# SerezD/vqvae-vqgan-pytorch-lightning

Measured on AMD Instinct MI355X. Metric: images/sec/node (256x256 bs=32/GPU) VQ-VAE train step, higher is better.
Workload: dtype bf16; 1 GPU; standard_vqvae cb=1024, 256x256 bs=32/GPU (encoder+VQ+decoder fwd/bwd + AdamW); yaml=example_confs/standard_vqvae.yaml, global_batch=32, parallelism=dp1, launch=hipGraph replay (fwd+bwd) + eager all-reduce + AdamW, deterministic=False

## Files before the change

### vqvae-vqgan-pytorch-lightning_amd/csrc/api.cpp

```cpp
#include <stdint.h>
#include <new>
#include "common.h"

extern "C" {

const char* vqk_status_str(int status) {
    switch (status) {
        case VQK_OK: return "ok";
        case VQK_ERR_SHAPE: return "unsupported or inconsistent shape";
        case VQK_ERR_DTYPE: return "unsupported dtype";
        case VQK_ERR_ALIGN: return "pointer is not 16-byte aligned";
        case VQK_ERR_LAUNCH: return "kernel launch failed";
        case VQK_ERR_ARG: return "bad argument";
        case VQK_ERR_WORKSPACE: return "workspace too small";
        default: return "unknown status";
    }
}

int vqk_version(void) { return 1; }
const char* vqk_arch(void) { return "gfx950"; }

}

struct vqk_ctx {
    vqkd::DetState det, scratch, tq;
};
namespace vqkd {
static vqk_ctx& default_ctx() {
    static thread_local vqk_ctx c = {{0, nullptr, 0}, {0, nullptr, 0}, {0, nullptr, 0}};
    return c;
}
static vqk_ctx*& current_ctx() {
    static thread_local vqk_ctx* cur = nullptr;
    return cur;
}
static vqk_ctx& ctx() {
    vqk_ctx* c = current_ctx();
    return c ? *c : default_ctx();
}
DetState& det_state() { return ctx().det; }
DetState& scratch_state() { return ctx().scratch; }
DetState& tile_queue_state() { return ctx().tq; }
}

extern "C" int vqk_ctx_create(vqk_ctx** out) {
    if (!out) return VQK_ERR_ARG;
    *out = new (std::nothrow) vqk_ctx{{0, nullptr, 0}, {0, nullptr, 0}, {0, nullptr, 0}};
    return *out ? VQK_OK : VQK_ERR_WORKSPACE;
}

extern "C" int vqk_ctx_destroy(vqk_ctx* c) {
    if (c && vqkd::current_ctx() == c) vqkd::current_ctx() = nullptr;
    delete c;
    return VQK_OK;
}

extern "C" int vqk_ctx_make_current(vqk_ctx* c) {
    vqkd::current_ctx() = c;
    return VQK_OK;
}

extern "C" int vqk_ctx_set_tile_queue(vqk_ctx* c, void* ws, int64_t ws_bytes) {
    if (ws && ws_bytes < 64) return VQK_ERR_WORKSPACE;
    if (ws && (reinterpret_cast<uintptr_t>(ws) & 15)) return VQK_ERR_ALIGN;
    vqkd::DetState& d = c ? c->tq : vqkd::ctx().tq;
    d.on = ws ? 1 : 0;
    d.ws = reinterpret_cast<float*>(ws);
    d.bytes = ws ? ws_bytes : 0;
    return VQK_OK;
}

extern "C" int vqk_ctx_set_scratch(vqk_ctx* c, void* ws, int64_t ws_bytes) {
    if (ws && ws_bytes < 0) return VQK_ERR_ARG;
    if (ws && (reinterpret_cast<uintptr_t>(ws) & 15)) return VQK_ERR_ALIGN;
    vqkd::DetState& d = c ? c->scratch : vqkd::ctx().scratch;
    d.on = ws ? 1 : 0;
    d.ws = reinterpret_cast<float*>(ws);
    d.bytes = ws ? ws_bytes : 0;
    return VQK_OK;
}

extern "C" int vqk_ctx_set_deterministic(vqk_ctx* c, int on, void* ws, int64_t ws_bytes) {
    if (on && ws && ws_bytes < 0) return VQK_ERR_ARG;
    if (on && ws && (reinterpret_cast<uintptr_t>(ws) & 15)) return VQK_ERR_ALIGN;
    vqkd::DetState& d = c ? c->det : vqkd::ctx().det;
    d.on = on ? 1 : 0;
    d.ws = (on && ws) ? reinterpret_cast<float*>(ws) : nullptr;
    d.bytes = (on && ws) ? ws_bytes : 0;
    return VQK_OK;
}

extern "C" int vqk_set_tile_queue(void* ws, int64_t ws_bytes) { return vqk_ctx_set_tile_queue(nullptr, ws, ws_bytes); }
extern "C" int vqk_set_scratch(void* ws, int64_t ws_bytes) { return vqk_ctx_set_scratch(nullptr, ws, ws_bytes); }
extern "C" int vqk_set_deterministic(int on, void* ws, int64_t ws_bytes) { return vqk_ctx_set_deterministic(nullptr, on, ws, ws_bytes); }

#include <string.h>
#include <stdlib.h>
namespace vqkd {
static TuneSlot g_tune[] = {
    {"MX", 0, 0},
    {"MX_1X1", 0, 0},
    {"TW16", 0, 0},
    {"STREAM_BLOCKS", 0, 0},
    {"MX_MIN_TILES", 0, 0},
    {"FPROP_SPLITK", 0, 0},
    {"SK_BLOCKS", 0, 0},
    {"SK_MINSTEPS", 0, 0},
    {"SK_MAXMB", 0, 0},
    {"UPS_PHASE", 0, 0},
    {"WGRAD_BLOCKS", 0, 0},
    {"WGMX", 0, 0},
    {"WGRAD_GEN_BLOCKS", 0, 0},
    {"WGRAD_NO_PW16", 0, 0},
    {"WGRAD_NO_P16K", 0, 0},
    {"MX_HALF", 0, 0},
    {"MX_HALF_HW", 0, 0},
    {"UPFIRDN_TILE", 0, 0},
    {"GN_BLOCKS_REDUCE", 0, 0},
    {"GN_BLOCKS_APPLY", 0, 0},
    {"GN_NT_MB", 0, 0},
    {"GN_NO_SMALL", 0, 0},
    {"WGMX_COEF_E4", 0, 0},
    {"GN_CLUSTER_MAX_HW", 0, 0},
    {"COMM_CUS", 0, 0},
    {"MX_QUARTER", 0, 0},
    {"MX_S2", 0, 0},
    {"MX_S2_DGRAD_MIN", 0, 0},
    {"VQ_LDS", 0, 0},
    {"UPS_MERGE", 0, 0},
    {"TILE_QUEUE", 0, 0},
    {"X3_WL", 0, 0},
    {"X3_WGRAD_COEF_E4", 0, 0},
    {"X3_WGRAD_FOLD", 0, 0},
    {"X3_WGRAD_PHASE", 0, 0},
    {"X3_WGRAD_PHASE_CAP_PCT", 0, 0},
    {"X3_WGRAD_PHASE_COEF_E4", 0, 0},
    {"WGRAD_GROUP_LOAD_PCT", 0, 0},
    {"WGRAD_GROUP_MIN_PPS", 0, 0},
    {"MX_PHASE_U64", 0, 0}
};
static constexpr int kTune = (int)(sizeof(g_tune) / sizeof(g_tune[0]));
TuneSlot* tune_slot(const char* name) {
    for (int i = 0; i < kTune; ++i)
        if (strcmp(g_tune[i].name, name) == 0) return &g_tune[i];
    abort();
}
}

extern "C" int vqk_set_tuning(const char* name, int value) {
    if (!name) return VQK_ERR_ARG;
    for (int i = 0; i < vqkd::kTune; ++i)
        if (strcmp(vqkd::g_tune[i].name, name) == 0) {
            __atomic_store_n(&vqkd::g_tune[i].value, value, __ATOMIC_RELAXED);
            __atomic_store_n(&vqkd::g_tune[i].is_set, 1, __ATOMIC_RELEASE);
            return VQK_OK;
        }
    return VQK_ERR_ARG;
}

extern "C" int vqk_reset_tuning(void) {
    for (int i = 0; i < vqkd::kTune; ++i) __atomic_store_n(&vqkd::g_tune[i].is_set, 0, __ATOMIC_RELAXED);
    return VQK_OK;
}

extern "C" int vqk_tuning_count(void) { return vqkd::kTune; }

extern "C" const char* vqk_tuning_name(int i) { return (i >= 0 && i < vqkd::kTune) ? vqkd::g_tune[i].name : nullptr; }
```

### vqvae-vqgan-pytorch-lightning_amd/csrc/conv_geom.h

```cpp
#pragma once
#include "common.h"

namespace vqkd {

struct ConvGeom {
    int n, h_in, w_in, h, w, cin, cout, ks, ups;
    int stride, pad, zs, vh, vw;
    float acc_scale, out_gain;
    int pool;
    float pool_scale;
    int m;
    int sub, sub_py, sub_px, sub_h, sub_w, nkh, nkw, khl[2], kwl[2];
    int wrow_chunks;
    int cpt;
    int kchunks;
    int tiles_m, tiles_n;
    int unit64;
    double* gn_ws;
    int gn_cpg;
    int gn_part_nblk, gn_part_base;
    int ntap, tap_oy, tap_ox, src_s, src_a, src_b, dst_s, dst_a, dst_b;
    int tapw, dst_h, dst_w, s2;
    int phase_mode;
    int phase_rev;
    int dy_pool;
    int act;
    int* tq;
    int tq_mode;
    int fold;
};

__device__ __forceinline__ int xcd_remap(int bid, int total) {
    const int q = total >> 3, r = total & 7, xcd = bid & 7, k = bid >> 3;
    return (xcd < r ? xcd * (q + 1) : r * (q + 1) + (xcd - r) * q) + k;
}

__device__ __forceinline__ unsigned pack_bf16x2(float a, float b) {
    typedef __attribute__((ext_vector_type(2))) float f32x2;
    typedef __attribute__((ext_vector_type(2))) __bf16 bf16x2_t;
    const f32x2 v = {a, b};
    return __builtin_bit_cast(unsigned, __builtin_convertvector(v, bf16x2_t));
}

constexpr int MX_LDS_MAX = 160 * 1024;
constexpr int mx_phase_u64_lds(int twlog) {
    return 2 * ((((256 >> twlog) + 1) * ((1 << twlog) + 1) * 9 + 63) / 64) * 1024 + 256 * 272 + 1024 + 64;
}

int launch_conv3x3_mx(const void* x, const void* w, const float* bias, const void* res, void* y, const void* zeros,
                      const ConvGeom& g, int twlog, hipStream_t st);

int conv_make_geom(ConvGeom& g, int dtype, int n, int h_in, int w_in, int cin, int cout, int ksize, int ups);
}
enum ConvVariant : int {
    CONV_VARIANT_AUTO = -1,
    CONV_VARIANT_IM2COL = 0,
    CONV_VARIANT_HALO = 1,
    CONV_VARIANT_PLAIN_WEIGHTS = 2,
    CONV_VARIANT_BREG = 3,
    CONV_VARIANT_NO_HALF = 4,
    CONV_VARIANT_NO_MX = 5,
    CONV_VARIANT_MX = 6,
};
enum WgradDyPool : int {
    WGRAD_DY_PLAIN = 0,
    WGRAD_DY_POOLED = 1,
    WGRAD_DY_PHASE0 = 2,
    WGRAD_DY_PHASES = 6,
    WGRAD_DY_PHASES_SWAPPED = 7,
};
enum WgradOp : int {
    WGRAD_OP_PLAIN = 0,
    WGRAD_OP_POOLED_DY = 1,
    WGRAD_OP_UPS_PHASE = 2,
    WGRAD_OP_POOLED_DY_PHASE = 3,
    WGRAD_OP_FOLD = 4,
    WGRAD_OP_X3 = 5,
};
namespace vqkd {
int& conv_force_variant();
int& conv_wgrad_blocks();

bool conv3x3_x3_serves(const ConvGeom& g);
int launch_conv3x3_x3(const void* x, const void* w, const float* bias, const void* res, void* y, const void* zeros,
                      const ConvGeom& g, int act, int blocks_cap, hipStream_t st);
int launch_conv3x3_wgrad_x3(const void* x, const void* dy, float* dw, const ConvGeom& g, int tiles, int splits, int pps, hipStream_t st);

int launch_conv3x3_thin_out_f32(const float* x, const float* w, const float* bias, const float* res, float* y, int n, int h, int wd,
                                int cin, int act, float acc_scale, float out_gain, hipStream_t st);
int launch_conv3x3_thin_in_f32(const float* x, const float* w, const float* bias, float* y, int n, int h, int wd, int cout, hipStream_t st);
int thin_wgrad_rows(int h, int w);
int launch_conv3x3_wgrad_thin_f32(int mode, const float* wide, const float* thin, float* dw, int n, int h, int w, int cw, float scale,
                                  hipStream_t st);

int launch_conv3x3_wgrad_mx(const void* x, const void* dy, float* dw, const void* zeros, const ConvGeom& g, int tiles,
                            int splits, int pps, hipStream_t st, float* part = nullptr);

#define VQK_WGRAD_GROUP_MAX 16
struct WgradGroupLayer {
    const void* x; const void* dy; float* dw;
    int n, h, w, cin, cout;
    float scale;
    int blk0, tiles, pps;
    int own;
};
struct WgradGroupTable {
    int n_layers, pad_;
    WgradGroupLayer layer[VQK_WGRAD_GROUP_MAX];
};
int launch_conv3x3_wgrad_mx_group(const WgradGroupTable& tb, int blocks, const void* zeros, hipStream_t st);

}
```

### vqvae-vqgan-pytorch-lightning_amd/csrc/conv_wgrad.hip

```cpp
#include "conv_geom.h"
#include <math.h>

namespace {

using vqkd::ConvGeom;
using vqkd::xcd_remap;

__device__ __forceinline__ void glds16(const void* src, char* lds_wave_base) {
    __builtin_amdgcn_global_load_lds((const VQK_GLB void*)src, (VQK_LDS void*)lds_wave_base, 16, 0, 0);
}

template <typename T> struct WgradFrag;

template <> struct WgradFrag<bf16_raw> {
    static constexpr int KP = 64;
    static constexpr int ROWB = 256;
    __device__ static __forceinline__ bf16x8_t frag(const char* tile, int k0, int cbase, int lane) {
        const int i = lane & 15, grp = (lane >> 4) & 1, kgrp = lane >> 5;
        const int col = cbase + 16 * grp + 4 * (i & 3);
        const int row = k0 + 8 * kgrp + (i >> 2);
        const int lc = col >> 3;
        const char* p0 = tile + row * ROWB + ((lc ^ ((row & 3) << 2)) << 4) + ((col & 7) << 1);
        const char* p1 = p0 + 4 * ROWB;
        const s16x4 lo = __builtin_amdgcn_ds_read_tr16_b64_v4i16((VQK_LDS s16x4*)p0);
// ... 437 lines not shown
    const int tco = bx / tiles_ci, tci = bx - tco * tiles_ci;
    const int co0 = tco * 64, ci0 = tci * 64;
    const int pw = g.w >> 4, ph = g.h >> 3;
    const int total_patches = g.n * ph * pw;
    const int p_begin = by * patches_per_split;
    const int p_end = min(total_patches, p_begin + patches_per_split);
    if (p_begin >= p_end) return;

    const int wi = wave >> 1, wj = wave & 1;
    f32x16 acc[9];
#pragma unroll
    for (int t = 0; t < 9; ++t)
#pragma unroll
        for (int r = 0; r < 16; ++r) acc[t][r] = 0.0f;

    const int lrow = lane >> 2, lch = (lane & 3) * 8;
    unsigned dyoff[NDY], xoff[NX];
#pragma unroll
    for (int sl = 0; sl < NDY; ++sl) {
        const int q = wave + 4 * sl, half = q >> 3, prow = q & 7;
        dyoff[sl] = (unsigned)((((prow * g.w + lrow) * g.cout) + co0 + half * 32 + lch) * 2);
    }
#pragma unroll
    for (int sl = 0; sl < NX; ++sl) {
        const int r = wave + 4 * sl, half = r / 12, row = min((r % 12) * 16 + lrow, HROWS - 1);
        const int hy = row / HWD, hx = row - hy * HWD;
        xoff[sl] = (unsigned)((((hy * g.w_in + hx) * g.cin) + ci0 + half * 32 + lch) * 2);
    }
    struct PatchPos { int img, py0, px0; bool interior; const char* bdy; const char* bx; };
    auto decode = [&](int patch) -> PatchPos {
        PatchPos pp;
        pp.img = patch / (ph * pw);
        const int rem = patch - pp.img * (ph * pw);
        const int pyi = rem / pw, pxi = rem - pyi * pw;
        pp.py0 = pyi * 8; pp.px0 = pxi * PWD;
        pp.interior = !g.ups && pp.py0 >= 1 && pp.py0 + 8 < g.h && pp.px0 >= 1 && pp.px0 + PWD < g.w;
        const int64_t pix = ((int64_t)pp.img * g.h + pp.py0) * g.w + pp.px0;
        pp.bdy = reinterpret_cast<const char*>(dy + pix * g.cout);
        pp.bx = reinterpret_cast<const char*>(x + (pix - g.w - 1) * g.cin);
        return pp;
    };
    auto piece = [&](bool interior, int sl, const PatchPos& pp, char* st) {
        if (sl < NDY) {
            const int q = wave + 4 * sl;
            char* dst = st + (q >> 3) * DY_HALF + (q & 7) * 1024;
            if (interior || true) {
                glds16(pp.bdy + dyoff[sl], dst);
            }
        } else {
            const int r = wave + 4 * (sl - NDY), half = r / 12, pr = r % 12;
            char* dst = st + 2 * DY_HALF + half * X_HALF + pr * 1024;
            if (interior) {
                glds16(pp.bx + xoff[sl - NDY], dst);
            } else {
                const int row = min(pr * 16 + lrow, HROWS - 1);
                const int hy = row / HWD, hx = row - hy * HWD;
                const int iy = pp.py0 + hy - 1, ix = pp.px0 + hx - 1;
                const void* src = zeros;
                if (iy >= 0 && iy < g.h && ix >= 0 && ix < g.w)
                    src = x + (((int64_t)pp.img * g.h_in + (iy >> g.ups)) * g.w_in + (ix >> g.ups)) * g.cin + ci0 + half * 32 + lch;
                glds16(src, dst);
            }
        }
    };

    const int li = lane & 15, grp = (lane >> 4) & 1, kgrp = lane >> 5;
    const unsigned frag_lane = (unsigned)((li >> 2) * 64 + 32 * grp + 8 * (li & 3));
    const unsigned a_lane = (unsigned)(wi * DY_HALF) + frag_lane + (unsigned)(kgrp * 8 * 64);
    const unsigned b_lane = (unsigned)(2 * DY_HALF + wj * X_HALF) + frag_lane + (unsigned)(kgrp * 8 * 64);

    {
        const PatchPos p0 = decode(p_begin);
#pragma unroll
        for (int sl = 0; sl < NDY + NX; ++sl) piece(p0.interior, sl, p0, smem);
    }
    for (int pch = p_begin; pch < p_end; ++pch) {
        const unsigned cur = (unsigned)(((pch - p_begin) & 1) * STAGE);
        asm volatile("s_waitcnt vmcnt(0)" ::: "memory");
        __syncthreads();
        const bool has_next = pch + 1 < p_end;
        const PatchPos pp = decode(has_next ? pch + 1 : pch);
        char* nst = smem + (STAGE - cur);
        const char* pa = smem + cur + a_lane;
        const char* pb = smem + cur + b_lane;
        if (has_next) {
            if (pp.interior) {
#pragma unroll
                for (int sl = 0; sl < NDY + NX; ++sl) piece(true, sl, pp, nst);
            } else {
#pragma unroll
                for (int sl = 0; sl < NDY + NX; ++sl) piece(false, sl, pp, nst);
            }
        }
        bf16x8_t bwin[3][3];
#pragma unroll
        for (int r = 0; r < 2; ++r)
#pragma unroll
            for (int tx = 0; tx < 3; ++tx) bwin[r][tx] = tr_frag2(pb + (r * HWD + tx) * 64);
#pragma unroll
        for (int gk = 0; gk < 8; ++gk) {
#pragma unroll
            for (int tx = 0; tx < 3; ++tx) bwin[(gk + 2) % 3][tx] = tr_frag2(pb + ((gk + 2) * HWD + tx) * 64);
            const bf16x8_t a = tr_frag2(pa + gk * 16 * 64);
#pragma unroll
            for (int t = 0; t < 9; ++t)
                acc[t] = __builtin_amdgcn_mfma_f32_32x32x16_bf16(a, bwin[(gk + t / 3) % 3][t % 3], acc[t], 0, 0, 0);
        }
    }
    const int ci = ci0 + wj * 32 + (lane & 31);
#pragma unroll
    for (int t = 0; t < 9; ++t)
#pragma unroll
        for (int r = 0; r < 16; ++r) {
            const int co = co0 + wi * 32 + (r & 3) + 8 * (r >> 2) + 4 * kgrp;
            atomicAdd(dw + ((int64_t)co * 9 + t) * g.cin + ci, acc[t][r] * g.acc_scale);
        }
}

__global__ __launch_bounds__(256) void wgrad_split_reduce_kernel(const float* __restrict__ part, int64_t elems, int splits,
                                                                 float* __restrict__ dw) {
    const int64_t i = (int64_t)blockIdx.x * 256 + threadIdx.x;
    if (i >= elems) return;
    float s = 0.f;
    for (int k = 0; k < splits; ++k) s += part[(int64_t)k * elems + i];
    dw[i] += s;
}

#define g_general_only (vqkd::conv_force_variant() == CONV_VARIANT_IM2COL)
#define g_wgrad_blocks (vqkd::conv_wgrad_blocks())
#define g_det (vqkd::det_state().on)
#define g_det_ws (vqkd::det_state().ws)
#define g_det_ws_bytes (vqkd::det_state().bytes)
inline int make_geom(ConvGeom& g, int dtype, int n, int h_in, int w_in, int cin, int cout, int ksize, int ups) {
    return vqkd::conv_make_geom(g, dtype, n, h_in, w_in, cin, cout, ksize, ups);
}

enum WgradForm : int {
    WGF_MX = 0,
    WGF_MX_POOLED_DY,
    WGF_MX_UPS_PHASE,
    WGF_MX_POOLED_DY_PHASE,
    WGF_MX_FOLD,
    WGF_P16,
    WGF_HALO16,
    WGF_HALO8,
    WGF_THIN_F32_CIN4,
    WGF_THIN_F32_COUT4,
    WGF_GENERAL_F32,
    WGF_GENERAL_BF16,
    WGF_GENERAL_DB,
    WGF_X3,
    WGF_X3_UPS_PHASE,
    WGF_X3_POOLED_PHASE,
    WGF_COUNT
};

struct WgradProblem {
    int op;
    int dtype, n, h_in, w_in, cin, cout, ksize, stride, pad, mode, h_out, w_out;
    float scale;
};
inline WgradProblem plain3x3(int op, int dtype, int n, int h, int w, int cin, int cout, int ups, float scale) {
    return {op, dtype, n, h, w, cin, cout, 3, 1, 1, ups, ups == 1 ? 2 * h : h, ups == 1 ? 2 * w : w, scale};
}

struct WgradPlan {
    int status;
    int form;
    int tiles;
    int splits;
    int pps;
    int launches;
    int ordered;
};
struct WgradSplit { int splits, pps; };

inline bool mx_wgrad_shape_ok(int h, int w, int cin, int cout) {
    return (h % 8) == 0 && (w % 16) == 0 && (cin % 64) == 0 && (cout % 64) == 0;
}
inline bool mx_wgrad_enabled(int op, bool grouped = false) {
    if (!VQK_TUNE("WGMX", 1) || g_general_only || VQK_TUNE("WGRAD_BLOCKS", 0) != 0 || VQK_TUNE("WGRAD_NO_PW16", 0) != 0) return false;
    if (g_det && (grouped || (op != WGRAD_OP_PLAIN && op != WGRAD_OP_POOLED_DY))) return false;
    return op != WGRAD_OP_POOLED_DY_PHASE || VQK_TUNE("UPS_MERGE", 1) != 0;
}

WgradSplit split_halo(int m, int tiles, int total_patches, bool pw16) {
    const int target = VQK_TUNE("WGRAD_BLOCKS", 0);
    const int cap = g_wgrad_blocks > 0 ? g_wgrad_blocks : 512;
    int splits;
    if (target > 0) splits = (target + tiles - 1) / tiles;
    else {
        splits = (int)(sqrt(0.16 * (double)m / tiles) + 0.5);
        if (splits > (cap + tiles - 1) / tiles) splits = (cap + tiles - 1) / tiles;
    }
    const int minp = pw16 ? 2 : 4;
    if (splits > (total_patches + minp - 1) / minp) splits = (total_patches + minp - 1) / minp;
    if (splits < 1 || g_det) splits = 1;
    const int pps = (total_patches + splits - 1) / splits;
    return {(total_patches + pps - 1) / pps, pps};
}

WgradSplit split_mx(int m, int tiles, int total_patches, int nph, int& ordered) {
    const int cap = g_wgrad_blocks > 0 ? g_wgrad_blocks : 512;
    const double coef = VQK_TUNE("WGMX_COEF_E4", 800) * 1e-4;
    const int comm = VQK_TUNE("COMM_CUS", 0);
    const int capm = (cap / 2 - comm) / nph > tiles ? (cap / 2 - comm) / nph : tiles;
    int sm = (int)(sqrt(coef * (double)m / tiles) + 0.5);
    if (sm > (capm + tiles - 1) / tiles) sm = (capm + tiles - 1) / tiles;
    if (sm > (total_patches + 3) / 4) sm = (total_patches + 3) / 4;
    if (g_det) {
        const int64_t per_split = (int64_t)tiles * 64 * 9 * 64 * 4;
        const int fit = (int)(g_det_ws_bytes / per_split);
        if (sm > fit) sm = fit;
    }
    if (sm < 1) sm = 1;
    const int ppm = (total_patches + sm - 1) / sm;
    sm = (total_patches + ppm - 1) / ppm;
    ordered = g_det && sm >= 2;
    return {sm, ppm};
}

WgradSplit split_general(int m, int tiles, int kp, bool db, int64_t dw_elems) {
    const int wg_target = VQK_TUNE("WGRAD_GEN_BLOCKS", 512);
    const int target_blocks = db ? wg_target : 2048;
    int splits = (target_blocks + tiles - 1) / tiles;
    const int max_splits = (m + 4 * kp - 1) / (4 * kp);
    if (splits > max_splits) splits = max_splits;
    if (g_det) {
        const int64_t fit = g_det_ws ? g_det_ws_bytes / (dw_elems * 4) : 0;
        if (splits > fit) splits = (int)fit;
    }
    if (splits < 1) splits = 1;
    int pps = (m + splits - 1) / splits;
    pps = ((pps + kp - 1) / kp) * kp;
    return {(m + pps - 1) / pps, pps};
}

WgradSplit split_x3(int m, int tiles, int total_patches, int phases) {
    int cap = g_wgrad_blocks > 0 ? g_wgrad_blocks : 512;
    if (phases == 4) cap = cap * VQK_TUNE("X3_WGRAD_PHASE_CAP_PCT", 150) / 100;
    const double coef = (phases == 4 ? VQK_TUNE("X3_WGRAD_PHASE_COEF_E4", 3200) : VQK_TUNE("X3_WGRAD_COEF_E4", 3200)) * 1e-4;
    int splits = (int)(sqrt(coef * (double)m * phases / tiles) / phases + 0.5);
    if (splits > (cap + tiles * phases - 1) / (tiles * phases)) splits = (cap + tiles * phases - 1) / (tiles * phases);
    if (splits > (total_patches + 3) / 4) splits = (total_patches + 3) / 4;
    if (splits < 1) splits = 1;
    const int pps = (total_patches + splits - 1) / splits;
    return {(total_patches + pps - 1) / pps, pps};
}

int wgrad_op_check(const WgradProblem& q) {
    if (q.op == WGRAD_OP_PLAIN || q.op == WGRAD_OP_X3) return VQK_OK;
    if (q.op == WGRAD_OP_FOLD) {
        VQK_REQUIRE(q.mode == 0 || q.mode == 1, VQK_ERR_ARG);
        VQK_REQUIRE((q.cin % 64) == 0 && (q.cout % 64) == 0, VQK_ERR_SHAPE);
        return VQK_OK;
    }
    VQK_REQUIRE(q.op == WGRAD_OP_POOLED_DY || q.op == WGRAD_OP_UPS_PHASE || q.op == WGRAD_OP_POOLED_DY_PHASE, VQK_ERR_ARG);
    VQK_REQUIRE(q.dtype == VQK_BF16 && mx_wgrad_shape_ok(q.h_in, q.w_in, q.cin, q.cout) && mx_wgrad_enabled(q.op), VQK_ERR_SHAPE);
    return VQK_OK;
}

WgradPlan plan_wgrad_x3(const WgradProblem& q, ConvGeom& g) {
    WgradPlan p = {VQK_OK, WGF_X3, 0, 1, 0, 1, 0};
    auto refuse = [&](int status) { p.status = status; return p; };
    const int ups = q.mode;
    if (ups != 0 && ups != 1 && ups != 2) return refuse(VQK_ERR_ARG);
    if (g_det || g_general_only) return refuse(VQK_ERR_SHAPE);
    const bool phase = ups == 2 || (ups == 1 && VQK_TUNE("X3_WGRAD_PHASE", 1) && (q.h_in % 8) == 0 && (q.w_in % 8) == 0);
    if (phase) {
        if (ups == 2 && ((q.h_in % 16) != 0 || (q.w_in % 16) != 0)) return refuse(VQK_ERR_SHAPE);
        const int rc = make_geom(g, VQK_F32, q.n, ups == 2 ? q.h_in / 2 : q.h_in, ups == 2 ? q.w_in / 2 : q.w_in, q.cin, q.cout, 3, 0);
        if (rc) return refuse(rc);
        g.ntap = 4; g.phase_mode = ups == 2 ? 2 : 1;
    } else {
        const int rc = make_geom(g, VQK_F32, q.n, q.h_in, q.w_in, q.cin, q.cout, 3, ups);
        if (rc) return refuse(rc);
    }
    g.acc_scale = q.scale;
    if ((g.cin & 63) || (g.cout & 63) || (g.h & 7) || (g.w & 7)) return refuse(VQK_ERR_SHAPE);
    p.form = !phase ? WGF_X3 : ups == 1 ? WGF_X3_UPS_PHASE : WGF_X3_POOLED_PHASE;
    p.tiles = (g.cout >> 6) * (g.cin >> 6);
    const WgradSplit s = split_x3(g.m, p.tiles, g.n * (g.h >> 3) * (g.w >> 3), phase ? 4 : 1);
    p.splits = s.splits; p.pps = s.pps;
    return p;
}

WgradPlan plan_wgrad(const WgradProblem& q, ConvGeom& g) {
    if (q.op == WGRAD_OP_X3) return plan_wgrad_x3(q, g);
    WgradPlan p = {VQK_OK, WGF_GENERAL_F32, 0, 1, 0, 1, 0};
    auto refuse = [&](int status) { p.status = status; return p; };
    auto take = [&](int form, int tiles, WgradSplit s) { p.form = form; p.tiles = tiles; p.splits = s.splits; p.pps = s.pps; return p; };
    const int rco = wgrad_op_check(q);
    if (rco) return refuse(rco);
    if (q.mode < 0 || q.mode > 1 || (q.stride != 1 && q.stride != 2) || q.pad < 0) return refuse(VQK_ERR_ARG);
    const bool fold = q.op == WGRAD_OP_FOLD, swapped = q.op == WGRAD_OP_POOLED_DY_PHASE;
    const int cin = fold ? 2 * q.cin : swapped ? q.cout : q.cin, cout = fold ? 2 * q.cout : swapped ? q.cin : q.cout;
    const int dtype = q.dtype, ksize = q.ksize;
    const int rc = make_geom(g, dtype, q.n, q.h_in, q.w_in, cin, cout, ksize, q.mode);
    if (rc) return refuse(rc);
    if (cout % (dtype == VQK_F32 ? 4 : 8)) return refuse(VQK_ERR_SHAPE);
    g.acc_scale = q.scale;
    const bool plain = q.stride == 1 && q.pad == (ksize >> 1) && q.h_out == g.h && q.w_out == g.w;
    if (!plain) {
        g.stride = q.stride; g.pad = q.pad;
        if (q.h_out <= 0 || q.w_out <= 0) return refuse(VQK_ERR_SHAPE);
        g.h = q.h_out; g.w = q.w_out;
        const int64_t m = (int64_t)q.n * q.h_out * q.w_out;
        if (m >= 0x7fffff00) return refuse(VQK_ERR_SHAPE);
        g.m = (int)m;
    }
    const bool bf3 = plain && dtype == VQK_BF16 && ksize == 3;
    if (bf3 && mx_wgrad_shape_ok(g.h, g.w, q.cin, q.cout) && mx_wgrad_enabled(q.op)) {
        static const int forms[] = {WGF_MX, WGF_MX_POOLED_DY, WGF_MX_UPS_PHASE, WGF_MX_POOLED_DY_PHASE, WGF_MX_FOLD};
        static const int dy_pools[] = {WGRAD_DY_PLAIN, WGRAD_DY_POOLED, WGRAD_DY_PHASES, WGRAD_DY_PHASES_SWAPPED, WGRAD_DY_PLAIN};
        const bool per_phase = q.op == WGRAD_OP_UPS_PHASE && !VQK_TUNE("UPS_MERGE", 1);
        g.dy_pool = per_phase ? (int)WGRAD_DY_PHASE0 : dy_pools[q.op];
        g.fold = fold;
        const int tiles = fold ? 3 * (cout / 128) * (cin / 128) : (cout / 64) * (cin / 64);
        const WgradSplit s = split_mx(g.m, tiles, g.n * (g.h / 8) * (g.w / 16), g.dy_pool >= WGRAD_DY_PHASES ? 4 : 1, p.ordered);
        p.launches = per_phase ? 4 : p.ordered ? 2 : 1;
        return take(forms[q.op], tiles, s);
    }
    if (q.op != WGRAD_OP_PLAIN) return refuse(VQK_ERR_SHAPE);
    if (bf3 && (g.h % 8) == 0 && (g.w % 8) == 0 && !g_general_only) {
        const bool pw16 = (g.w % 16) == 0 && VQK_TUNE("WGRAD_NO_PW16", 0) == 0;
        const int tiles = ((cout + 63) / 64) * ((cin + 63) / 64);
        const WgradSplit s = split_halo(g.m, tiles, g.n * (g.h / 8) * (g.w / (pw16 ? 16 : 8)), pw16);
        if (pw16 && (cin % 64) == 0 && (cout % 64) == 0 && VQK_TUNE("WGRAD_NO_P16K", 0) == 0) return take(WGF_P16, tiles, s);
        return take(pw16 ? WGF_HALO16 : WGF_HALO8, tiles, s);
    }
    if (plain && dtype == VQK_F32 && ksize == 3 && q.mode == 0 && !g_det && !g_general_only && (g.w % 4) == 0) {
        const int rows = vqkd::thin_wgrad_rows(g.h, g.w);
        auto wide = [](int c) { return c == 64 || c == 128 || c == 256; };
        if (rows > 0 && cin == 4 && wide(cout)) return take(WGF_THIN_F32_CIN4, g.n * (g.h / rows), {1, rows});
        if (rows > 0 && cout == 4 && wide(cin)) return take(WGF_THIN_F32_COUT4, g.n * (g.h / rows), {1, rows});
    }
    const bool db = dtype == VQK_BF16 && ksize == 1;
    const int tiles = ((cout + 127) / 128) * ((cin + 127) / 128) * ksize * ksize;
    const WgradSplit s = split_general(g.m, tiles, dtype == VQK_F32 ? 32 : 64, db, (int64_t)cout * ksize * ksize * cin);
    p.ordered = g_det && s.splits > 1;
    p.launches = p.ordered ? 2 : 1;
    return take(dtype == VQK_F32 ? WGF_GENERAL_F32 : db ? WGF_GENERAL_DB : WGF_GENERAL_BF16, tiles, s);
}

template <auto KERNEL, int LDS>
void launch_patch(const WgradPlan& p, const ConvGeom& g, const void* x, const void* dy, float* dw, const void* zeros, hipStream_t st) {
    static const hipError_t attr = LDS > 65536 ? hipFuncSetAttribute((const void*)KERNEL, hipFuncAttributeMaxDynamicSharedMemorySize, LDS)
                                               : hipSuccess;
    (void)attr;
    hipLaunchKernelGGL(KERNEL, dim3((unsigned)p.tiles, (unsigned)p.splits), dim3(256), LDS, st, (const bf16_raw*)x, (const bf16_raw*)dy, dw,
                       (const char*)zeros, g, p.pps);
}
template <typename T>
void launch_general(const WgradPlan& p, const ConvGeom& g, const void* x, const void* dy, float* dst, int64_t sstride, const void* zeros,
                    hipStream_t st) {
    const int taps = g.ks * g.ks;
    hipLaunchKernelGGL(conv_wgrad_kernel<T>, dim3((unsigned)(p.tiles / taps), (unsigned)taps, (unsigned)p.splits), dim3(256), 32768, st,
                       (const T*)x, (const T*)dy, dst, (const char*)zeros, g, p.pps, sstride);
}
int launch_general_db(const WgradPlan& p, const ConvGeom& g, const void* x, const void* dy, float* dst, int64_t sstride, const void* zeros,
                      hipStream_t st) {
    static const hipError_t attr = hipFuncSetAttribute((const void*)conv_wgrad_db_kernel, hipFuncAttributeMaxDynamicSharedMemorySize, 65536);
    if (attr != hipSuccess) return VQK_ERR_LAUNCH;
    hipLaunchKernelGGL(conv_wgrad_db_kernel, dim3((unsigned)p.tiles, 1, (unsigned)p.splits), dim3(256), 65536, st, (const bf16_raw*)x,
                       (const bf16_raw*)dy, dst, (const char*)zeros, g, p.pps, sstride);
    return VQK_OK;
}

int launch_wgrad(const WgradPlan& p, const ConvGeom& g, const void* x, const void* dy, float* dw, const void* zeros, hipStream_t st) {
    if (p.status != VQK_OK) return p.status;
    switch (p.form) {
    case WGF_MX:
    case WGF_MX_POOLED_DY:
    case WGF_MX_FOLD:
        return vqkd::launch_conv3x3_wgrad_mx(x, dy, dw, zeros, g, p.tiles, p.splits, p.pps, st, p.ordered ? g_det_ws : nullptr);
    case WGF_MX_POOLED_DY_PHASE:
        return vqkd::launch_conv3x3_wgrad_mx(dy, x, dw, zeros, g, p.tiles, 4 * p.splits, p.pps, st);
    case WGF_MX_UPS_PHASE: {
        if (p.launches == 1) return vqkd::launch_conv3x3_wgrad_mx(x, dy, dw, zeros, g, p.tiles, 4 * p.splits, p.pps, st);
        ConvGeom gp = g;
        for (int ph = 0; ph < p.launches; ++ph) {
            gp.dy_pool = WGRAD_DY_PHASE0 + ph;
            const int rc = vqkd::launch_conv3x3_wgrad_mx(x, dy, dw, zeros, gp, p.tiles, p.splits, p.pps, st);
            if (rc) return rc;
        }
        return VQK_OK;
    }
    case WGF_P16: launch_patch<conv3x3_wgrad_p16_kernel, 2 * 40960>(p, g, x, dy, dw, zeros, st); break;
    case WGF_HALO16: launch_patch<conv3x3_wgrad_halo_kernel<true>, 2 * 40960>(p, g, x, dy, dw, zeros, st); break;
    case WGF_HALO8: launch_patch<conv3x3_wgrad_halo_kernel<false>, 2 * 22528>(p, g, x, dy, dw, zeros, st); break;
    case WGF_THIN_F32_CIN4:
        return vqkd::launch_conv3x3_wgrad_thin_f32(0, (const float*)dy, (const float*)x, dw, g.n, g.h, g.w, g.cout, g.acc_scale, st);
    case WGF_THIN_F32_COUT4:
        return vqkd::launch_conv3x3_wgrad_thin_f32(1, (const float*)x, (const float*)dy, dw, g.n, g.h, g.w, g.cin, g.acc_scale, st);
    case WGF_GENERAL_F32:
    case WGF_GENERAL_BF16:
    case WGF_GENERAL_DB: {
        const int64_t dw_elems = (int64_t)g.cout * g.ks * g.ks * g.cin;
        float* dst = p.ordered ? g_det_ws : dw;
        const int64_t sstride = p.ordered ? dw_elems : 0;
        if (p.ordered && hipMemsetAsync(dst, 0, (size_t)p.splits * dw_elems * 4, st) != hipSuccess) return VQK_ERR_LAUNCH;
        if (p.form == WGF_GENERAL_F32) launch_general<float>(p, g, x, dy, dst, sstride, zeros, st);
        else if (p.form == WGF_GENERAL_BF16) launch_general<bf16_raw>(p, g, x, dy, dst, sstride, zeros, st);
        else if (launch_general_db(p, g, x, dy, dst, sstride, zeros, st)) return VQK_ERR_LAUNCH;
        if (p.ordered)
            hipLaunchKernelGGL(wgrad_split_reduce_kernel, dim3((unsigned)((dw_elems + 255) / 256)), dim3(256), 0, st, (const float*)dst,
                               dw_elems, p.splits, dw);
        break;
    }
    case WGF_X3:
    case WGF_X3_UPS_PHASE:
    case WGF_X3_POOLED_PHASE:
        return vqkd::launch_conv3x3_wgrad_x3(x, dy, dw, g, p.tiles, p.splits, p.pps, st);
    default: return VQK_ERR_ARG;
    }
    VQK_CHECK_LAUNCH();
    return VQK_OK;
}

}

extern "C" {

static int wgrad_run(const WgradProblem& q, const void* x, const void* dy, float* dw, const void* zeros, void* stream) {
    const int rc = wgrad_op_check(q);
    if (rc) return rc;
    VQK_REQUIRE(x && dy && dw && zeros, VQK_ERR_ARG);
    VQK_REQUIRE(vqk_aligned16(x) && vqk_aligned16(dy) && vqk_aligned16(zeros), VQK_ERR_ALIGN);
    ConvGeom g;
    const WgradPlan p = plan_wgrad(q, g);
    return launch_wgrad(p, g, x, dy, dw, zeros, vqk_stream(stream));
}

int vqk_conv2d_wgrad(int dtype, const void* x, const void* dy, float* dw, int n, int h_in, int w_in, int cin, int cout,
                     int ksize, int ups, const void* zeros, void* stream) {
    VQK_REQUIRE(ups == 0 || ups == 1, VQK_ERR_ARG);
    return wgrad_run({WGRAD_OP_PLAIN, dtype, n, h_in, w_in, cin, cout, ksize, 1, ksize >> 1, ups, h_in << ups, w_in << ups, 1.0f}, x, dy,
                     dw, zeros, stream);
}

int vqk_conv2d_wgrad_general(int dtype, const void* x, const void* dy, float* dw, int n, int h_in, int w_in, int cin,
                             int cout, int ksize, int stride, int pad, int mode, int h_out, int w_out, const void* zeros,
                             void* stream) {
    return wgrad_run({WGRAD_OP_PLAIN, dtype, n, h_in, w_in, cin, cout, ksize, stride, pad, mode, h_out, w_out, 1.0f}, x, dy, dw, zeros,
                     stream);
}

int vqk_conv2d_wgrad_general_scaled(int dtype, const void* x, const void* dy, float* dw, int n, int h_in, int w_in, int cin,
                                    int cout, int ksize, int stride, int pad, int mode, int h_out, int w_out, float scale,
                                    const void* zeros, void* stream) {
    return wgrad_run({WGRAD_OP_PLAIN, dtype, n, h_in, w_in, cin, cout, ksize, stride, pad, mode, h_out, w_out, scale}, x, dy, dw, zeros,
                     stream);
}

int vqk_conv2d_wgrad_pooled_dy(int dtype, const void* x, const void* dy_pooled, float* dw, int n, int h, int w, int cin,
                               int cout, float scale, const void* zeros, void* stream) {
    return wgrad_run(plain3x3(WGRAD_OP_POOLED_DY, dtype, n, h, w, cin, cout, 0, scale), x, dy_pooled, dw, zeros, stream);
}

int vqk_conv2d_wgrad_ups_phase(int dtype, const void* x, const void* dy, float* dw, int n, int h, int w, int cin, int cout,
                                float scale, const void* zeros, void* stream) {
    return wgrad_run(plain3x3(WGRAD_OP_UPS_PHASE, dtype, n, h, w, cin, cout, 0, scale), x, dy, dw, zeros, stream);
}

int vqk_conv2d_wgrad_pooled_dy_phase(int dtype, const void* x, const void* dy_pooled, float* dw, int n, int h, int w, int cin,
                                     int cout, float scale, const void* zeros, void* stream) {
    return wgrad_run(plain3x3(WGRAD_OP_POOLED_DY_PHASE, dtype, n, h, w, cin, cout, 0, scale), x, dy_pooled, dw, zeros, stream);
}

int vqk_conv2d_wgrad_x3(const void* x_pair, const void* dy_pair, float* dw, int n, int h_in, int w_in, int cin, int cout, int ups,
                        float scale, const void* zeros, void* stream) {
    return wgrad_run(plain3x3(WGRAD_OP_FOLD, VQK_BF16, n, h_in, w_in, cin, cout, ups, scale), x_pair, dy_pair, dw, zeros, stream);
}

int vqk_conv2d_wgrad_x3_f32(const float* x, const float* dy, float* dw, int n, int h_in, int w_in, int cin, int cout, int ups,
                            float scale, void* stream) {
    VQK_REQUIRE(x && dy && dw, VQK_ERR_ARG);
    VQK_REQUIRE(vqk_aligned16(x) && vqk_aligned16(dy), VQK_ERR_ALIGN);
    ConvGeom g;
    const WgradPlan p = plan_wgrad({WGRAD_OP_X3, VQK_F32, n, h_in, w_in, cin, cout, 3, 1, 1, ups, 0, 0, scale}, g);
    return launch_wgrad(p, g, x, dy, dw, nullptr, vqk_stream(stream));
}

int vqk_conv_wgrad_plan(int op, int dtype, int n, int h_in, int w_in, int cin, int cout, int ksize, int stride, int pad, int ups,
                        int h_out, int w_out, int* details) {
    VQK_REQUIRE(op >= WGRAD_OP_PLAIN && op <= WGRAD_OP_X3, VQK_ERR_ARG);
    ConvGeom g;
    WgradProblem q = {op, dtype, n, h_in, w_in, cin, cout, ksize, stride, pad, ups, h_out, w_out, 1.0f};
    if (op == WGRAD_OP_X3) q.dtype = VQK_F32;
    else if (op != WGRAD_OP_PLAIN) q = plain3x3(op, op == WGRAD_OP_FOLD ? (int)VQK_BF16 : dtype, n, h_in, w_in, cin, cout, op == WGRAD_OP_FOLD ? ups : 0, 1.0f);
    const WgradPlan p = plan_wgrad(q, g);
    if (p.status != VQK_OK) return p.status;
    if (details) {
        details[0] = p.tiles; details[1] = p.splits; details[2] = p.pps; details[3] = p.launches;
        details[4] = p.form == WGF_THIN_F32_CIN4 || p.form == WGF_THIN_F32_COUT4;
    }
    return p.form;
}

const char* vqk_conv_wgrad_form_name(int form, int dtype) {
    static const char* const names[WGF_COUNT] = {
        "conv3x3_wgrad_mx_kernel<bf16>", "conv3x3_wgrad_mx_kernel<bf16>", "conv3x3_wgrad_mx_kernel<bf16>", "conv3x3_wgrad_mx_kernel<bf16>",
        "conv3x3_wgrad_mx_kernel<f32 as 3 x bf16>", "conv3x3_wgrad_p16_kernel<bf16>", "conv3x3_wgrad_halo_kernel<bf16>",
        "conv3x3_wgrad_halo_kernel<bf16>", "conv3x3_wgrad_thin_f32_kernel (HBM)", "conv3x3_wgrad_thin_f32_kernel (HBM)",
        "conv_wgrad_kernel<f32>", "conv_wgrad_kernel<bf16>", "conv_wgrad_db_kernel<bf16>", "conv3x3_wgrad_x3_kernel<f32 as 3 x bf16>",
        "conv3x3_wgrad_x3_kernel<f32 as 3 x bf16>", "conv3x3_wgrad_x3_kernel<f32 as 3 x bf16>",
    };
    if (form < 0 || form >= WGF_COUNT || (dtype != VQK_F32 && dtype != VQK_BF16)) return "?";
    return names[form];
}


static int wgrad_group_plan(const vqk_wgrad_item* it, int n, int* splits, int* pps) {
    const int load_pct = VQK_TUNE("WGRAD_GROUP_LOAD_PCT", 150), min_pps = VQK_TUNE("WGRAD_GROUP_MIN_PPS", 4);
    VQK_REQUIRE(load_pct >= 1 && min_pps >= 1, VQK_ERR_ARG);
    int64_t work = 0;
    for (int i = 0; i < n; ++i) work += (int64_t)(it[i].cout / 64) * (it[i].cin / 64) * ((int64_t)it[i].n * (it[i].h / 8) * (it[i].w / 16));
    int64_t len = work * load_pct / (256 * 100);
    if (len < min_pps) len = min_pps;
    for (int i = 0; i < n; ++i) {
        const int patches = it[i].n * (it[i].h / 8) * (it[i].w / 16);
        int s = (int)((patches + len - 1) / len);
        if (s < 1) s = 1;
        pps[i] = (patches + s - 1) / s;
        splits[i] = (patches + pps[i] - 1) / pps[i];
    }
    return VQK_OK;
}

static int wgrad_group_check(const vqk_wgrad_item* items, int n_items) {
    VQK_REQUIRE(items && n_items >= 1, VQK_ERR_ARG);
    VQK_REQUIRE(mx_wgrad_enabled(WGRAD_OP_PLAIN, true), VQK_ERR_SHAPE);
    for (int i = 0; i < n_items; ++i) {
        const vqk_wgrad_item& q = items[i];
        VQK_REQUIRE(q.x && q.dy && q.dw, VQK_ERR_ARG);
        VQK_REQUIRE(q.dtype == VQK_BF16 && q.ksize == 3 && q.ups == 0 && q.n >= 1 && q.h >= 8 && q.w >= 16 && q.cin >= 64 && q.cout >= 64
                    && mx_wgrad_shape_ok(q.h, q.w, q.cin, q.cout), VQK_ERR_SHAPE);
        VQK_REQUIRE((int64_t)q.n * q.h * q.w < 0x7fffff00 && (int64_t)q.n * q.h * q.w * (q.cin > q.cout ? q.cin : q.cout) < (1ll << 31),
                    VQK_ERR_SHAPE);
        VQK_REQUIRE(vqk_aligned16(q.x) && vqk_aligned16(q.dy) && vqk_aligned16(q.dw), VQK_ERR_ALIGN);
    }
    return VQK_OK;
}

int vqk_conv3x3_wgrad_group_plan(const vqk_wgrad_item* items, int n_items, int* splits, int* launches) {
    const int rc = wgrad_group_check(items, n_items);
    if (rc) return rc;
    VQK_REQUIRE(splits && launches, VQK_ERR_ARG);
    *launches = (n_items + VQK_WGRAD_GROUP_MAX - 1) / VQK_WGRAD_GROUP_MAX;
    int pps[VQK_WGRAD_GROUP_MAX];
    for (int i0 = 0; i0 < n_items; i0 += VQK_WGRAD_GROUP_MAX) {
        const int n = n_items - i0 < VQK_WGRAD_GROUP_MAX ? n_items - i0 : VQK_WGRAD_GROUP_MAX;
        const int rp = wgrad_group_plan(items + i0, n, splits + i0, pps);
        if (rp) return rp;
    }
    return VQK_OK;
}

int vqk_conv3x3_wgrad_group(const vqk_wgrad_item* items, int n_items, const void* zeros, void* stream) {
    const int rc = wgrad_group_check(items, n_items);
    if (rc) return rc;
    VQK_REQUIRE(zeros, VQK_ERR_ARG);
    VQK_REQUIRE(vqk_aligned16(zeros), VQK_ERR_ALIGN);
    for (int i0 = 0; i0 < n_items; i0 += VQK_WGRAD_GROUP_MAX) {
        const vqk_wgrad_item* it = items + i0;
        const int n = n_items - i0 < VQK_WGRAD_GROUP_MAX ? n_items - i0 : VQK_WGRAD_GROUP_MAX;
        int splits[VQK_WGRAD_GROUP_MAX], pps[VQK_WGRAD_GROUP_MAX], order[VQK_WGRAD_GROUP_MAX];
        const int rp = wgrad_group_plan(it, n, splits, pps);
        if (rp) return rp;
        for (int i = 0; i < n; ++i) {
            int j = i;
            for (; j > 0 && pps[order[j - 1]] < pps[i]; --j) order[j] = order[j - 1];
            order[j] = i;
        }
        vqkd::WgradGroupTable tb = {};
        tb.n_layers = n;
        int blocks = 0;
        for (int k = 0; k < n; ++k) {
            const int i = order[k];
            vqkd::WgradGroupLayer& L = tb.layer[k];
            L.x = it[i].x; L.dy = it[i].dy; L.dw = it[i].dw;
            L.n = it[i].n; L.h = it[i].h; L.w = it[i].w; L.cin = it[i].cin; L.cout = it[i].cout;
            L.scale = it[i].scale;
            L.blk0 = blocks; L.tiles = (it[i].cout / 64) * (it[i].cin / 64); L.pps = pps[i];
            L.own = splits[i] == 1;
            for (int j = 0; j < n; ++j)
                if (j != i && it[j].dw == it[i].dw) L.own = 0;
            blocks += L.tiles * splits[i];
        }
        const int rl = vqkd::launch_conv3x3_wgrad_mx_group(tb, blocks, zeros, vqk_stream(stream));
        if (rl) return rl;
    }
    return VQK_OK;
}

}
```

Before: 1224 images/sec.

## Add warp-specialized streaming 1x1 conv weight-gradient kernel with sqrt-based split planning

Result: no change. 1228 images/sec (median of 6 runs) (+0.3%).

```diff
diff --git a/vqvae-vqgan-pytorch-lightning_amd/csrc/api.cpp b/vqvae-vqgan-pytorch-lightning_amd/csrc/api.cpp
--- a/vqvae-vqgan-pytorch-lightning_amd/csrc/api.cpp
+++ b/vqvae-vqgan-pytorch-lightning_amd/csrc/api.cpp
@@ -137,7 +137,9 @@
     {"X3_WGRAD_PHASE_COEF_E4", 0, 0},
     {"WGRAD_GROUP_LOAD_PCT", 0, 0},
     {"WGRAD_GROUP_MIN_PPS", 0, 0},
-    {"MX_PHASE_U64", 0, 0}
+    {"MX_PHASE_U64", 0, 0},
+    {"WG1X1", 0, 0},
+    {"WG1X1_COEF_E4", 0, 0}
 };
 static constexpr int kTune = (int)(sizeof(g_tune) / sizeof(g_tune[0]));
 TuneSlot* tune_slot(const char* name) {
diff --git a/vqvae-vqgan-pytorch-lightning_amd/csrc/conv_geom.h b/vqvae-vqgan-pytorch-lightning_amd/csrc/conv_geom.h
--- a/vqvae-vqgan-pytorch-lightning_amd/csrc/conv_geom.h
+++ b/vqvae-vqgan-pytorch-lightning_amd/csrc/conv_geom.h
@@ -110,4 +110,7 @@
 };
 int launch_conv3x3_wgrad_mx_group(const WgradGroupTable& tb, int blocks, const void* zeros, hipStream_t st);
 
+int launch_conv1x1_wgrad_stream(const void* x, const void* dy, float* dw, const void* zeros, const ConvGeom& g, int tiles, int splits,
+                                int pps, hipStream_t st);
+
 }
diff --git a/vqvae-vqgan-pytorch-lightning_amd/csrc/conv_wg1x1.hip b/vqvae-vqgan-pytorch-lightning_amd/csrc/conv_wg1x1.hip
--- /dev/null
+++ b/vqvae-vqgan-pytorch-lightning_amd/csrc/conv_wg1x1.hip
@@ -0,0 +1,150 @@
+#include "conv_geom.h"
+
+namespace {
+using vqkd::xcd_remap;
+
+constexpr int KP = 64;
+constexpr int NST = 4, LEAD = NST - 1;
+constexpr int HALF = KP * 64;
+constexpr int OPER = 4 * HALF;
+constexpr int STAGE = 2 * OPER;
+constexpr int NPIECE = 8;
+static_assert(NST == 4 && KP == 64, "stage index masks and the wave -> row-group map below");
+
+__device__ __forceinline__ void glds16(const void* src, char* lds_wave_base) {
+    __builtin_amdgcn_global_load_lds((const VQK_GLB void*)src, (VQK_LDS void*)lds_wave_base, 16, 0, 0);
+}
+__device__ __forceinline__ bf16x8_t tr_frag2(const char* p) {
+    const s16x4 lo = __builtin_amdgcn_ds_read_tr16_b64_v4i16((VQK_LDS s16x4*)p);
+    const s16x4 hi = __builtin_amdgcn_ds_read_tr16_b64_v4i16((VQK_LDS s16x4*)(p + 256));
+    typedef __attribute__((ext_vector_type(8))) short s16x8;
+    const s16x8 v = {lo[0], lo[1], lo[2], lo[3], hi[0], hi[1], hi[2], hi[3]};
+    return __builtin_bit_cast(bf16x8_t, v);
+}
+
+__global__ __launch_bounds__(512) void conv1x1_wgrad_stream_kernel(const bf16_raw* __restrict__ x, const bf16_raw* __restrict__ dy,
+                                                                   float* __restrict__ dw, const char* __restrict__ zeros, int m,
+                                                                   int cin, int cout, float scale, int pps) {
+    extern __shared__ __attribute__((aligned(16))) char smem[];
+    const int tid = threadIdx.x, lane = tid & 63;
+    const int wave = __builtin_amdgcn_readfirstlane(tid >> 6);
+    const int tiles_ci = cin >> 7, tiles = tiles_ci * (cout >> 7);
+    const int vb = xcd_remap((int)blockIdx.x, (int)gridDim.x);
+    const int split = vb / tiles, tile = vb - split * tiles;
+    const int tco = tile / tiles_ci, tci = tile - tco * tiles_ci;
+    const int co0 = tco * 128, ci0 = tci * 128;
+    const int p_begin = split * pps;
+    const int p_end = min(m, p_begin + pps);
+    if (p_begin >= p_end) return;
+    const int nstage = (p_end - p_begin + KP - 1) / KP;
+    const bool own = (int)gridDim.x == tiles;
+
+    const int last = nstage - 1;
+    auto stage_barrier = [&]() { asm volatile("s_waitcnt lgkmcnt(0)\n\ts_barrier" ::: "memory"); };
+
+    if (wave >= 4) {
+        const int xw = wave - 4;
+        const int lrow = 16 * xw + (lane >> 2), lch = (lane & 3) * 8;
+        const char* sdy = reinterpret_cast<const char*>(dy + (int64_t)(p_begin + lrow) * cout + co0 + lch);
+        const char* sx = reinterpret_cast<const char*>(x + (int64_t)(p_begin + lrow) * cin + ci0 + lch);
+        const int64_t step_dy = (int64_t)KP * cout * 2, step_x = (int64_t)KP * cin * 2;
+        auto issue = [&](int s) {
+            char* st = smem + (s & 3) * STAGE + xw * 1024;
+            const bool ok = p_begin + s * KP + lrow < p_end;
+            const char* a = ok ? sdy + s * step_dy : zeros;
+            const char* b = ok ? sx + s * step_x : zeros;
+            const int hs = ok ? 64 : 0;
+#pragma unroll
+            for (int h = 0; h < 4; ++h) glds16(a + h * hs, st + h * HALF);
+#pragma unroll
+            for (int h = 0; h < 4; ++h) glds16(b + h * hs, st + OPER + h * HALF);
+        };
+        auto wait_stages = [&](int k) {
+            if (k >= 2) asm volatile("s_waitcnt vmcnt(16)" ::: "memory");
+            else if (k == 1) asm volatile("s_waitcnt vmcnt(8)" ::: "memory");
+            else asm volatile("s_waitcnt vmcnt(0)" ::: "memory");
+        };
+        static_assert(NPIECE == 8 && LEAD == 3, "the counts of wait_stages");
+#pragma unroll
+        for (int k = 0; k < LEAD; ++k)
+            if (k <= last) issue(k);
+        wait_stages(min(last, LEAD - 1));
+        stage_barrier();
+        for (int s = 0; s <= last; ++s) {
+            if (s + LEAD <= last) issue(s + LEAD);
+            wait_stages(s + 1 <= last ? min(last, s + LEAD) - (s + 1) : 0);
+            stage_barrier();
+        }
+        return;
+    }
+
+    const int wm = wave >> 1, wn = wave & 1;
+    const int li = lane & 15, grp = (lane >> 4) & 1, kgrp = lane >> 5;
+    const unsigned frag_lane = (unsigned)((li >> 2) * 64 + 32 * grp + 8 * (li & 3) + kgrp * 8 * 64);
+    const unsigned a_lane = (unsigned)(2 * wm * HALF) + frag_lane;
+    const unsigned b_lane = (unsigned)(OPER + 2 * wn * HALF) + frag_lane;
+    f32x16 acc[2][2];
+#pragma unroll
+    for (int i = 0; i < 2; ++i)
+#pragma unroll
+        for (int j = 0; j < 2; ++j)
+#pragma unroll
+            for (int r = 0; r < 16; ++r) acc[i][j][r] = 0.0f;
+    stage_barrier();
+    for (int s = 0; s <= last; ++s) {
+        const char* pa = smem + (s & 3) * STAGE + a_lane;
+        const char* pb = smem + (s & 3) * STAGE + b_lane;
+#pragma unroll
+        for (int kk = 0; kk < KP / 16; ++kk) {
+            bf16x8_t a[2], b[2];
+#pragma unroll
+            for (int i = 0; i < 2; ++i) {
+                a[i] = tr_frag2(pa + i * HALF + kk * 1024);
+                b[i] = tr_frag2(pb + i * HALF + kk * 1024);
+            }
+#pragma unroll
+            for (int i = 0; i < 2; ++i)
+#pragma unroll
+                for (int j = 0; j < 2; ++j)
+                    acc[i][j] = __builtin_amdgcn_mfma_f32_32x32x16_bf16(a[i], b[j], acc[i][j], 0, 0, 0);
+        }
+        stage_barrier();
+    }
+
+    float* dtile = dw + (int64_t)(co0 + wm * 64 + 4 * kgrp) * cin + ci0 + wn * 64 + (lane & 31);
+#pragma unroll
+    for (int i = 0; i < 2; ++i)
+#pragma unroll
+        for (int j = 0; j < 2; ++j) {
+            float* d = dtile + (int64_t)(i * 32) * cin + j * 32;
+            if (own) {
+                float old[16];
+#pragma unroll
+                for (int r = 0; r < 16; ++r) old[r] = d[(int64_t)((r & 3) + 8 * (r >> 2)) * cin];
+#pragma unroll
+                for (int r = 0; r < 16; ++r) d[(int64_t)((r & 3) + 8 * (r >> 2)) * cin] = old[r] + acc[i][j][r] * scale;
+            } else {
+#pragma unroll
+                for (int r = 0; r < 16; ++r) atomicAdd(d + (int64_t)((r & 3) + 8 * (r >> 2)) * cin, acc[i][j][r] * scale);
+            }
+        }
+}
+
+}
+
+namespace vqkd {
+
+int launch_conv1x1_wgrad_stream(const void* x, const void* dy, float* dw, const void* zeros, const ConvGeom& g, int tiles, int splits,
+                                int pps, hipStream_t st) {
+    if (g.ks != 1 || (g.cin & 127) || (g.cout & 127) || tiles != (g.cin >> 7) * (g.cout >> 7) || splits < 1 || pps < 1
+        || (int64_t)splits * pps < g.m)
+        return VQK_ERR_ARG;
+    static const hipError_t attr = hipFuncSetAttribute((const void*)conv1x1_wgrad_stream_kernel,
+                                                       hipFuncAttributeMaxDynamicSharedMemorySize, NST * STAGE);
+    if (attr != hipSuccess) return VQK_ERR_LAUNCH;
+    hipLaunchKernelGGL(conv1x1_wgrad_stream_kernel, dim3((unsigned)(tiles * splits)), dim3(512), NST * STAGE, st, (const bf16_raw*)x,
+                       (const bf16_raw*)dy, dw, (const char*)zeros, g.m, g.cin, g.cout, g.acc_scale, pps);
+    return hipGetLastError() == hipSuccess ? VQK_OK : VQK_ERR_LAUNCH;
+}
+
+}
diff --git a/vqvae-vqgan-pytorch-lightning_amd/csrc/conv_wgrad.hip b/vqvae-vqgan-pytorch-lightning_amd/csrc/conv_wgrad.hip
--- a/vqvae-vqgan-pytorch-lightning_amd/csrc/conv_wgrad.hip
+++ b/vqvae-vqgan-pytorch-lightning_amd/csrc/conv_wgrad.hip
@@ -613,6 +613,7 @@
     WGF_X3,
     WGF_X3_UPS_PHASE,
     WGF_X3_POOLED_PHASE,
+    WGF_1X1_STREAM,
     WGF_COUNT
 };
 
@@ -707,6 +708,19 @@
     if (splits < 1) splits = 1;
     const int pps = (total_patches + splits - 1) / splits;
     return {(total_patches + pps - 1) / pps, pps};
+}
+
+WgradSplit split_1x1(int m, int tiles) {
+    constexpr int kp = 64, min_stages = 4;
+    const int cap = g_wgrad_blocks > 0 ? g_wgrad_blocks : 512;
+    const double coef = VQK_TUNE("WG1X1_COEF_E4", 1200) * 1e-4;
+    int s = (int)(sqrt(coef * (double)m / tiles) + 0.5);
+    if (s > cap / 2 / tiles) s = cap / 2 / tiles;
+    if (s > m / (min_stages * kp)) s = m / (min_stages * kp);
+    if (s < 1) s = 1;
+    int pps = (m + s - 1) / s;
+    pps = ((pps + kp - 1) / kp) * kp;
+    return {(m + pps - 1) / pps, pps};
 }
 
 int wgrad_op_check(const WgradProblem& q) {
@@ -797,7 +811,11 @@
         if (rows > 0 && cout == 4 && wide(cin)) return take(WGF_THIN_F32_COUT4, g.n * (g.h / rows), {1, rows});
     }
     const bool db = dtype == VQK_BF16 && ksize == 1;
-    const int tiles = ((cout + 127) / 128) * ((cin + 127) / 128) * ksize * ksize;
+    if (db && plain && q.mode == 0 && (cin % 128) == 0 && (cout % 128) == 0 && !g_det && !g_general_only && VQK_TUNE("WG1X1", 1)) {
+        const int t1 = (cout / 128) * (cin / 128);
+        return take(WGF_1X1_STREAM, t1, split_1x1(g.m, t1));
+    }
+    const int tiles =((cout + 127) / 128) * ((cin + 127) / 128) * ksize * ksize;
     const WgradSplit s = split_general(g.m, tiles, dtype == VQK_F32 ? 32 : 64, db, (int64_t)cout * ksize * ksize * cin);
     p.ordered = g_det && s.splits > 1;
     p.launches = p.ordered ? 2 : 1;
@@ -873,6 +891,8 @@
     case WGF_X3_UPS_PHASE:
     case WGF_X3_POOLED_PHASE:
         return vqkd::launch_conv3x3_wgrad_x3(x, dy, dw, g, p.tiles, p.splits, p.pps, st);
+    case WGF_1X1_STREAM:
+        return vqkd::launch_conv1x1_wgrad_stream(x, dy, dw, zeros, g, p.tiles, p.splits, p.pps, st);
     default: return VQK_ERR_ARG;
     }
     VQK_CHECK_LAUNCH();
@@ -954,7 +974,7 @@
     if (p.status != VQK_OK) return p.status;
     if (details) {
         details[0] = p.tiles; details[1] = p.splits; details[2] = p.pps; details[3] = p.launches;
-        details[4] = p.form == WGF_THIN_F32_CIN4 || p.form == WGF_THIN_F32_COUT4;
+        details[4] = p.form == WGF_THIN_F32_CIN4 || p.form == WGF_THIN_F32_COUT4 || p.form == WGF_1X1_STREAM;
     }
     return p.form;
 }
@@ -965,7 +985,7 @@
         "conv3x3_wgrad_mx_kernel<f32 as 3 x bf16>", "conv3x3_wgrad_p16_kernel<bf16>", "conv3x3_wgrad_halo_kernel<bf16>",
         "conv3x3_wgrad_halo_kernel<bf16>", "conv3x3_wgrad_thin_f32_kernel (HBM)", "conv3x3_wgrad_thin_f32_kernel (HBM)",
         "conv_wgrad_kernel<f32>", "conv_wgrad_kernel<bf16>", "conv_wgrad_db_kernel<bf16>", "conv3x3_wgrad_x3_kernel<f32 as 3 x bf16>",
-        "conv3x3_wgrad_x3_kernel<f32 as 3 x bf16>", "conv3x3_wgrad_x3_kernel<f32 as 3 x bf16>",
+        "conv3x3_wgrad_x3_kernel<f32 as 3 x bf16>", "conv3x3_wgrad_x3_kernel<f32 as 3 x bf16>", "conv1x1_wgrad_stream_kernel<bf16> (HBM)",
     };
     if (form < 0 || form >= WGF_COUNT || (dtype != VQK_F32 && dtype != VQK_BF16)) return "?";
     return names[form];
```
